# ipl-uw/ZeDO-Release

Measured on AMD Instinct MI355X. Metric: poses/sec (1000-step sampler, H=50), higher is better.
Workload: dtype f32; 1 GPU; BASELINE configs[2] (3DPW pw3d_test, H=50, 1000 steps): N=1015 poses/GPU x H=50 hypotheses, IPO 500 it (17 joints) + 1000 OIL steps + P1/P2 min-over-hypotheses selection; random-init ScoreModelFC_Adv weights, synthetic detections; settings=pw3d, rows_per_gpu=50750, poses_total=1015

## Files before the change

### zedo-release_amd/csrc/zedo_geom.hip

```cpp
#include "zedo_internal.h"

#include <atomic>
#include <cstdlib>

namespace zedo {


__global__ void pack_rows_kernel(const float *__restrict__ x, float *__restrict__ xpad, int B, int Bp, int D) {
    const size_t i = (size_t)blockIdx.x * blockDim.x + threadIdx.x;
    if (i >= (size_t)Bp * XLD) return;
    const int r = (int)(i / XLD), c = (int)(i % XLD);
#ifdef ZEDO_MUT_PACK51
    if (D > 51) D = 51;
#endif
    xpad[i] = (r < B && c < D) ? x[(size_t)r * D + c] : 0.0f;
}

__global__ void unpack_rows_kernel(const float *__restrict__ xpad, float *__restrict__ x, int B, int D) {
    const size_t i = (size_t)blockIdx.x * blockDim.x + threadIdx.x;
    if (i >= (size_t)B * D) return;
    const int r = (int)(i / D), c = (int)(i % D);
    x[i] = xpad[(size_t)r * XLD + c];
}

hipError_t launch_pack_rows(const float *x, float *xpad, int B, int Bp, int D, hipStream_t st) {
    const size_t n = (size_t)Bp * XLD;
    hipLaunchKernelGGL(pack_rows_kernel, dim3((unsigned)((n + 255) / 256)), dim3(256), 0, st, x, xpad, B, Bp, D);
    return hipGetLastError();
}
hipError_t launch_unpack_rows(const float *xpad, float *x, int B, int D, hipStream_t st) {
    const size_t n = (size_t)B * D;
    hipLaunchKernelGGL(unpack_rows_kernel, dim3((unsigned)((n + 255) / 256)), dim3(256), 0, st, xpad, x, B, D);
    return hipGetLastError();
}

__device__ __forceinline__ void inv3x3(const float *K, double *Ki) {
    const double a = K[0], b = K[1], c = K[2], d = K[3], e = K[4], f = K[5], g = K[6], h = K[7], i = K[8];
    const double A = e * i - f * h, Bc = -(d * i - f * g), C = d * h - e * g;
    const double det = a * A + b * Bc + c * C;
    const double id = 1.0 / det;
    Ki[0] = A * id;  Ki[1] = -(b * i - c * h) * id;  Ki[2] = (b * f - c * e) * id;
    Ki[3] = Bc * id; Ki[4] = (a * i - c * g) * id;   Ki[5] = -(a * f - c * d) * id;
    Ki[6] = C * id;  Ki[7] = -(a * h - b * g) * id;  Ki[8] = (a * e - b * d) * id;
}

__global__ void reproj_prepare_kernel(const float *__restrict__ uv, const float *__restrict__ K,
                                      const float *__restrict__ conf, int N, int J, float *__restrict__ geom,
                                      float *__restrict__ conf_out) {
    const int i = blockIdx.x * blockDim.x + threadIdx.x;
    if (i >= N * J) return;
    const int n = i / J;
    double Ki[9];
    inv3x3(K + (size_t)n * 9, Ki);
    const double u = uv[(size_t)i * 2], v = uv[(size_t)i * 2 + 1];
    const double rz = Ki[6] * u + Ki[7] * v + Ki[8];
    const double rx = (Ki[0] * u + Ki[1] * v + Ki[2]) / rz;
    const double ry = (Ki[3] * u + Ki[4] * v + Ki[5]) / rz;
    const double rn = 1.0 / sqrt(rx * rx + ry * ry + 1.0);
    float W = 1.0f;
    if (conf) {
        float c = conf[i];
        if (c > 1.0f) c = 1.0f;
        if (c < 1e-4f) c = 1e-4f;
        if (conf_out) conf_out[i] = c;
        const float w = c * c;
        W = w * w;
#ifdef ZEDO_MUT_CONF2
        W = w;
#endif
    }
    float *g = geom + (size_t)i * GEOM_F;
    g[0] = (float)rx; g[1] = (float)ry; g[2] = W; g[3] = 0.0f;
    g[4] = (float)(rx * rn); g[5] = (float)(ry * rn); g[6] = (float)rn; g[7] = 0.0f;
}

hipError_t launch_reproj_prepare(const float *uv, const float *K, const float *conf, int N, int J, float *geom,
                                 float *conf_clamped, hipStream_t st) {
    const int n = N * J;
    hipLaunchKernelGGL(reproj_prepare_kernel, dim3((n + 255) / 256), dim3(256), 0, st, uv, K, conf, N, J, geom,
                       conf_clamped);
    return hipGetLastError();
}

__global__ void reproj_degenerate_kernel(const float *__restrict__ geom, int N, int J, int *__restrict__ count) {
    const int n = blockIdx.x * blockDim.x + threadIdx.x;
    if (n >= N) return;
    const float *gp = geom + (size_t)n * J * GEOM_F;
    float sw = 0.f, srx = 0.f, sry = 0.f;
    for (int j = 0; j < J; ++j) {
        const f32x4 a = *reinterpret_cast<const f32x4 *>(gp + j * GEOM_F);
        sw += a[2]; srx += a[2] * a[0]; sry += a[2] * a[1];
    }
    const float iw = 1.0f / sw;
    const float mrx = srx * iw, mry = sry * iw;
    float den = 0.f;
    for (int j = 0; j < J; ++j) {
        const f32x4 a = *reinterpret_cast<const f32x4 *>(gp + j * GEOM_F);
        const float dx = a[0] - mrx, dy = a[1] - mry;
        den += a[2] * (dx * dx + dy * dy);
    }
    if (den == 0.f) atomicAdd(count, 1);
}

hipError_t launch_reproj_degenerate(const float *geom, int N, int J, int *d_count, hipStream_t st) {
    hipLaunchKernelGGL(reproj_degenerate_kernel, dim3((N + 255) / 256), dim3(256), 0, st, geom, N, J, d_count);
    return hipGetLastError();
}


template <int J>
__global__ __launch_bounds__(128) void reproj_grad_kernel(const float *__restrict__ x, const float *__restrict__ geom,
                                                          float *__restrict__ T, int solve, float *__restrict__ gout,
                                                          int B, int N, long long row_offset) {
    constexpr int D = J * 3, R = 128;
    __shared__ float sx[R * D];
    const int row0 = blockIdx.x * R, tid = threadIdx.x;
    const int rows = min(R, B - row0);
    const float *src = x + (size_t)row0 * D;
    for (int i = tid; i < rows * D; i += R) sx[i] = src[i];
    __syncthreads();
    float xr[D], gr[D], Tr[3];
    if (tid < rows) {
        const int b = row0 + tid;
#pragma unroll
        for (int c = 0; c < D; ++c) xr[c] = sx[tid * D + c];
        Tr[0] = T[(size_t)b * 3]; Tr[1] = T[(size_t)b * 3 + 1]; Tr[2] = T[(size_t)b * 3 + 2];
#ifdef ZEDO_MUT_RGRAD_OFFSET
        const int n = b % N;
#else
        const int n = (int)((row_offset + b) % N);
#endif
        reproj_row<J>(xr, geom + (size_t)n * J * GEOM_F, Tr, solve != 0, gr);
        if (solve) { T[(size_t)b * 3] = Tr[0]; T[(size_t)b * 3 + 1] = Tr[1]; T[(size_t)b * 3 + 2] = Tr[2]; }
    }
    __syncthreads();
    if (tid < rows) {
#pragma unroll
        for (int c = 0; c < D; ++c) sx[tid * D + c] = gr[c];
    }
    __syncthreads();
    float *dst = gout + (size_t)row0 * D;
    for (int i = tid; i < rows * D; i += R) dst[i] = sx[i];
}

hipError_t launch_reproj_grad(const float *x, const float *geom, float *T, int solve_T, float *g, int B, int N,
                              int J, long long row_offset, hipStream_t st) {
    if (J != 17) return hipErrorInvalidValue;
    hipLaunchKernelGGL(reproj_grad_kernel<17>, dim3((B + 127) / 128), dim3(128), 0, st, x, geom, T, solve_T, g, B, N,
                       row_offset);
    return hipGetLastError();
}

constexpr int TILE_LD = XLD + 4;
__device__ __forceinline__ void tile_to_lds(float *sx, const float *base, const int tid) {
#pragma unroll
    for (int it = 0; it < XLD / 4; ++it) {
        const int idx = it * BATCH_PAD + tid, r = idx >> 4, c4 = idx & 15;
        *reinterpret_cast<f32x4 *>(sx + r * TILE_LD + c4 * 4) = *reinterpret_cast<const f32x4 *>(base + (size_t)idx * 4);
    }
}
__device__ __forceinline__ void tile_from_lds(float *base, const float *sx, const int tid) {
#pragma unroll
    for (int it = 0; it < XLD / 4; ++it) {
        const int idx = it * BATCH_PAD + tid, r = idx >> 4, c4 = idx & 15;
        *reinterpret_cast<f32x4 *>(base + (size_t)idx * 4) = *reinterpret_cast<const f32x4 *>(sx + r * TILE_LD + c4 * 4);
    }
}

template <int J>
__global__ __launch_bounds__(64) void reproj_step_kernel(float *__restrict__ xpad, const float *__restrict__ geom,
                                                         float *__restrict__ T, int solve, int B, int N,
                                                         long long row_offset) {
    __shared__ __attribute__((aligned(16))) float sx[BATCH_PAD * TILE_LD];
    const int row0 = blockIdx.x * BATCH_PAD, tid = threadIdx.x;
    float *base = xpad + (size_t)row0 * XLD;
    tile_to_lds(sx, base, tid);
    __syncthreads();
    const int b = row0 + tid;
    if (b < B) ZEDO_REPROJ_STAGED_ROW(J, sx + tid * TILE_LD, 0, b, (ReprojArgs{geom, T, solve, B, N, row_offset}));
    __syncthreads();
    tile_from_lds(base, sx, tid);
}

template <int J>
__global__ __launch_bounds__(64) void post_reduce_kernel(float *__restrict__ xpad, const float *__restrict__ partial,
                                                         const float *__restrict__ bias, float sde_a, float sde_c, int sde,
                                                         float *__restrict__ eps_out, const float *__restrict__ geom,
                                                         float *__restrict__ T, int solve, int B, int N, long long row_offset) {
    __shared__ __attribute__((aligned(16))) float sx[BATCH_PAD * TILE_LD];
    __shared__ __attribute__((aligned(16))) float sb[XLD];
    const int row0 = blockIdx.x * BATCH_PAD, tid = threadIdx.x;
    float *base = (sde ? xpad : eps_out) + (size_t)row0 * XLD;
    sb[tid] = bias[tid];
    if (sde) tile_to_lds(sx, base, tid);
    __syncthreads();
    const int b = row0 + tid;
    {
        const float *p0 = partial + ((size_t)(b >> 5) * 4 * 32 + (b & 31)) * XLD;
        float *xr = sx + tid * TILE_LD;
#pragma unroll
        for (int v = 0; v < XLD / 4; ++v) {
            const f32x4 q0 = *reinterpret_cast<const f32x4 *>(p0 + v * 4);
            const f32x4 q1 = *reinterpret_cast<const f32x4 *>(p0 + 32 * XLD + v * 4);
            const f32x4 q2 = *reinterpret_cast<const f32x4 *>(p0 + 2 * 32 * XLD + v * 4);
#ifdef ZEDO_MUT_POST_Q3
            const f32x4 q3 = q2;
#else
            const f32x4 q3 = *reinterpret_cast<const f32x4 *>(p0 + 3 * 32 * XLD + v * 4);
#endif
            const f32x4 bb = *reinterpret_cast<const f32x4 *>(sb + v * 4);
            f32x4 x4 = {0.f, 0.f, 0.f, 0.f};
            if (sde) x4 = *reinterpret_cast<const f32x4 *>(xr + v * 4);
            f32x4 o;
#pragma unroll
            for (int e = 0; e < 4; ++e) {
                float t = ((q0[e] + q1[e]) + q2[e]) + q3[e];
                t = t + bb[e];
                if (sde) { t = t * sde_c; t = __builtin_fmaf(sde_a, x4[e], t); }
                o[e] = t;
            }
            *reinterpret_cast<f32x4 *>(xr + v * 4) = o;
        }
    }
    if (geom != nullptr && b < B) ZEDO_REPROJ_STAGED_ROW(J, sx + tid * TILE_LD, 0, b, (ReprojArgs{geom, T, solve, B, N, row_offset}));
    __syncthreads();
    tile_from_lds(base, sx, tid);
}

hipError_t launch_post_reduce(float *xpad, const float *partial, const float *bias, float sde_a, float sde_c, int sde,
                              float *eps_out, const ReprojArgs &rp, int Bp, hipStream_t st) {
    if (Bp % BATCH_PAD || !partial || !bias || (sde ? !xpad : !eps_out)) return hipErrorInvalidValue;
    hipLaunchKernelGGL(post_reduce_kernel<17>, dim3(Bp / BATCH_PAD), dim3(BATCH_PAD), 0, st, xpad, partial, bias, sde_a, sde_c, sde,
                       eps_out, rp.geom, rp.T, rp.solve, rp.B, rp.N > 0 ? rp.N : 1, rp.row0);
    return hipGetLastError();
}

hipError_t launch_reproj_step_padded(float *xpad, const ReprojArgs &rp, hipStream_t st) {
    hipLaunchKernelGGL(reproj_step_kernel<17>, dim3((rp.B + BATCH_PAD - 1) / BATCH_PAD), dim3(BATCH_PAD), 0, st, xpad, rp.geom, rp.T,
                       rp.solve, rp.B, rp.N, rp.row0);
    return hipGetLastError();
}

__global__ void posemb_kernel(const float *__restrict__ t, int S, int Sp, float label_scale, float *__restrict__ pe) {
    const int i = blockIdx.x * blockDim.x + threadIdx.x;
    if (i >= Sp * EMB) return;
    const int s = i / EMB, c = i % EMB;
    float o = 0.0f;
    if (s < S) {
        constexpr int half = EMB / 2;
        const float emb = (float)(-9.210340371976184 / (half - 1));
        const int k = c < half ? c : c - half;
        const float freq = expf((float)k * emb);
        const float arg = (t[s] * label_scale) * freq;
        o = c < half ? sinf(arg) : cosf(arg);
#ifdef ZEDO_MUT_POSEMB_FAST
        o = c < half ? __sinf(arg) : __cosf(arg);
#endif
    }
    pe[i] = o;
}

hipError_t launch_posemb(const float *t, int S, int Sp, float label_scale, float *pe, hipStream_t st) {
    const int n = Sp * EMB;
    hipLaunchKernelGGL(posemb_kernel, dim3((n + 255) / 256), dim3(256), 0, st, t, S, Sp, label_scale, pe);
    return hipGetLastError();
}

struct AdamP {
    float p, m, v;
    __device__ __forceinline__ void step(float g, float step_size, float bc2_sqrt) {
        m = m + (g - m) * 0.1f;
        v = v * 0.999f + 0.001f * g * g;
        const float denom = sqrtf(v) / bc2_sqrt + 1e-8f;
        p = p + (-step_size * m) / denom;
    }
};

__device__ __forceinline__ float sgnf(float e) { return (e > 0.f) ? 1.f : ((e < 0.f) ? -1.f : 0.f); }

constexpr int IPO_KMAX = 17;
static_assert(IPO_KMAX == 17, "launch_ipo_fit instantiates ipo_row_kernel<1 .. 17>: a longer key list needs its cases");
constexpr int IPO_TABLE = 2048;

struct IpoKeys { int j[IPO_KMAX]; };

__constant__ float c_adam_step[IPO_TABLE] = {
#define ZEDO_ADAM_STEP
#include "zedo_adam_table.inc"
#undef ZEDO_ADAM_STEP
};
__constant__ float c_adam_bc2s[IPO_TABLE] = {
#define ZEDO_ADAM_BC2S
#include "zedo_adam_table.inc"
#undef ZEDO_ADAM_BC2S
};

template <int M>
__device__ __forceinline__ float swz_xor(float v) {
    return __int_as_float(__builtin_amdgcn_ds_swizzle(__float_as_int(v), (M << 10) | 0x1F));
}
template <int CTRL>
__device__ __forceinline__ float dpp(float v) {
    return __int_as_float(__builtin_amdgcn_update_dpp(0, __float_as_int(v), CTRL, 0xF, 0xF, false));
}
template <int C>
__device__ __forceinline__ float bcast(float v) {
    return __int_as_float(__builtin_amdgcn_ds_swizzle(__float_as_int(v), (C << 5)));
}
__device__ __forceinline__ float half_sum(float v) {
    v = v + dpp<0x140>(v);
    v = v + dpp<0x141>(v);
    v = v + dpp<0x4E>(v);
    v = v + dpp<0xB1>(v);
    v = v + swz_xor<16>(v);
    return v;
}

struct IpoRot { float R00, R01, R02, R10, R11, R12, R20, R21, R22, Tx, Ty, Tz, ts; };

__device__ __forceinline__ IpoRot ipo_rot(float r, float i, float j, float kk, float scp, float min_s, float max_s, const float (&T0)[3]) {
    IpoRot o;
    const float n2 = r * r + i * i + j * j + kk * kk;
    const float ts = 2.0f / n2;
    o.ts = ts;
    o.R00 = 1.f - ts * (j * j + kk * kk); o.R01 = ts * (i * j - kk * r); o.R02 = ts * (i * kk + j * r);
    o.R10 = ts * (i * j + kk * r); o.R11 = 1.f - ts * (i * i + kk * kk); o.R12 = ts * (j * kk - i * r);
    o.R20 = ts * (i * kk - j * r); o.R21 = ts * (j * kk + i * r); o.R22 = 1.f - ts * (i * i + j * j);
    const float scc = fminf(fmaxf(scp, min_s), max_s);
    o.Tx = T0[0] * scc; o.Ty = T0[1] * scc; o.Tz = T0[2] * scc;
    return o;
}

__device__ __forceinline__ void ipo_joint_terms(const float (&K)[9], const float (&T0)[3], const IpoRot &o, float x, float y, float z,
                                                float cu, float cv, float inv_norm, float (&t)[10]) {
    const float px = o.R00 * x + o.R01 * y + o.R02 * z + o.Tx;
    const float py = o.R10 * x + o.R11 * y + o.R12 * z + o.Ty;
    const float pz = o.R20 * x + o.R21 * y + o.R22 * z + o.Tz;
    const float w0 = K[0] * px + K[1] * py + K[2] * pz;
    const float w1 = K[3] * px + K[4] * py + K[5] * pz;
#ifdef ZEDO_MUT_IPO_W2_K6
    const float w2 = K[7] * py + K[8] * pz;
#else
    const float w2 = K[6] * px + K[7] * py + K[8] * pz;
#endif
    const float gu = sgnf(w0 / w2 - cu) * inv_norm;
    const float gv = sgnf(w1 / w2 - cv) * inv_norm;
    const float gw0 = gu / w2, gw1 = gv / w2;
    const float gw2 = -gu * ((w0 / w2) / w2) - gv * ((w1 / w2) / w2);
    const float gpx = K[0] * gw0 + K[3] * gw1 + K[6] * gw2;
#ifdef ZEDO_MUT_IPO_GPY_K1
    const float gpy = K[4] * gw1 + K[7] * gw2;
#else
    const float gpy = K[1] * gw0 + K[4] * gw1 + K[7] * gw2;
#endif
    const float gpz = K[2] * gw0 + K[5] * gw1 + K[8] * gw2;
    t[0] = gpx * T0[0] + gpy * T0[1] + gpz * T0[2];
    t[1] = gpx * x; t[2] = gpx * y; t[3] = gpx * z;
    t[4] = gpy * x; t[5] = gpy * y; t[6] = gpy * z;
    t[7] = gpz * x; t[8] = gpz * y; t[9] = gpz * z;
}

__device__ __forceinline__ void ipo_quat_grads(const float (&S)[10], float r, float i, float j, float kk, float ts, float &gr, float &gi,
                                               float &gj, float &gk) {
    const float G00 = S[1], G01 = S[2], G02 = S[3], G10 = S[4], G11 = S[5], G12 = S[6], G20 = S[7], G21 = S[8], G22 = S[9];
    const float gts = G00 * -(j * j + kk * kk) + G01 * (i * j - kk * r) + G02 * (i * kk + j * r) +
                      G10 * (i * j + kk * r) + G11 * -(i * i + kk * kk) + G12 * (j * kk - i * r) +
                      G20 * (i * kk - j * r) + G21 * (j * kk + i * r) + G22 * -(i * i + j * j);
    const float dts = -gts * ts * ts;
    gr = ts * (-G01 * kk + G02 * j + G10 * kk - G12 * i - G20 * j + G21 * i) + dts * r;
    gi = ts * (G01 * j + G02 * kk + G10 * j - 2.f * G11 * i - G12 * r + G20 * kk + G21 * r - 2.f * G22 * i) + dts * i;
    gj = ts * (-2.f * G00 * j + G01 * i + G02 * r + G10 * i + G12 * kk - G20 * r + G21 * kk - 2.f * G22 * j) + dts * j;
    gk = ts * (-2.f * G00 * kk - G01 * r + G02 * i + G10 * r - 2.f * G11 * kk + G12 * j + G20 * i + G21 * j) + dts * kk;
}

__device__ __forceinline__ void ipo_T0(const float (&K)[9], double u, double v, float ipo_T, float (&T0)[3]) {
    double Ki[9];
    inv3x3(K, Ki);
    const double tx = Ki[0] * u + Ki[1] * v + Ki[2], ty = Ki[3] * u + Ki[4] * v + Ki[5], tz = Ki[6] * u + Ki[7] * v + Ki[8];
    const double in = (double)ipo_T / sqrt(tx * tx + ty * ty + tz * tz);
    T0[0] = (float)(tx * in); T0[1] = (float)(ty * in); T0[2] = (float)(tz * in);
}

__device__ __forceinline__ void ipo_adam_terms(int ta, double &b1p, double &b2p, float &step_size, float &bc2s) {
    b1p *= 0.9; b2p *= 0.999;
    if (ta < IPO_TABLE) { step_size = c_adam_step[ta]; bc2s = c_adam_bc2s[ta]; }
    else { step_size = (float)(0.1 / (1.0 - b1p)); bc2s = (float)sqrt(1.0 - b2p); }
}

__device__ __forceinline__ void ipo_store(const AdamP &qr, const AdamP &qi, const AdamP &qj, const AdamP &qk, const AdamP &sc, const float (&T0)[3],
                                          float min_s, float max_s, int b, float *Rout, float *Tout, float *qout, float *sout, float *stp) {
    const float r = qr.p, i = qi.p, j = qj.p, kk = qk.p;
    const float ts = 2.0f / (r * r + i * i + j * j + kk * kk);
    float *Ro = Rout + (size_t)b * 9;
    Ro[0] = 1.f - ts * (j * j + kk * kk); Ro[1] = ts * (i * j - kk * r); Ro[2] = ts * (i * kk + j * r);
    Ro[3] = ts * (i * j + kk * r); Ro[4] = 1.f - ts * (i * i + kk * kk); Ro[5] = ts * (j * kk - i * r);
    Ro[6] = ts * (i * kk - j * r); Ro[7] = ts * (j * kk + i * r); Ro[8] = 1.f - ts * (i * i + j * j);
    const float scc = fminf(fmaxf(sc.p, min_s), max_s);
    Tout[(size_t)b * 3] = T0[0] * scc; Tout[(size_t)b * 3 + 1] = T0[1] * scc; Tout[(size_t)b * 3 + 2] = T0[2] * scc;
    if (qout) { qout[(size_t)b * 4] = r; qout[(size_t)b * 4 + 1] = i; qout[(size_t)b * 4 + 2] = j; qout[(size_t)b * 4 + 3] = kk; }
    if (sout) sout[b] = sc.p;
    if (stp) {
        stp[0] = qr.p; stp[1] = qi.p; stp[2] = qj.p; stp[3] = qk.p; stp[4] = sc.p;
        stp[5] = qr.m; stp[6] = qi.m; stp[7] = qj.m; stp[8] = qk.m; stp[9] = sc.m;
#ifdef ZEDO_MUT_IPO_STORE_V
        stp[10] = qr.v; stp[11] = qi.v; stp[12] = qj.v; stp[13] = qk.v; stp[14] = sc.m;
#else
        stp[10] = qr.v; stp[11] = qi.v; stp[12] = qj.v; stp[13] = qk.v; stp[14] = sc.v;
#endif
    }
}

__global__ __launch_bounds__(64) void ipo_kernel(const float *__restrict__ x0, const float *__restrict__ uv,
                                                  const float *__restrict__ Kmat, const IpoKeys keylist,
                                                  int k, int axes_mask, float ipo_T, float min_s, float max_s,
                                                  int iters, float inv_norm, float *__restrict__ Rout,
                                                  float *__restrict__ Tout, float *__restrict__ qout,
                                                  float *__restrict__ sout, float *__restrict__ state,
                                                  int it_begin, double b1p0, double b2p0, int B, int N, int J,
                                                  long long row_offset) {
    __shared__ int s_kl[32];
    const int lane = threadIdx.x, jl = lane & 31;
    if (lane < 32) s_kl[lane] = lane < k ? keylist.j[lane] : keylist.j[0];
    __syncthreads();
    const int b_raw = blockIdx.x * 2 + (lane >> 5);
    const bool row_ok = b_raw < B;
    const int b = row_ok ? b_raw : B - 1;
#ifdef ZEDO_MUT_IPO_JOINT
    const bool jact = jl < k && jl < 16;
#else
    const bool jact = jl < k;
#endif
    const long long gb = row_offset + b;
    const int n = (int)(gb % N), h = (int)(gb / N);
    const int jn = s_kl[jl];
    const float *xh = x0 + ((size_t)h * J + jn) * 3;
    const float x = xh[0], y = xh[1], z = xh[2];
    const float cu = uv[((size_t)n * J + jn) * 2], cv = uv[((size_t)n * J + jn) * 2 + 1];
    float K[9];
#pragma unroll
    for (int i = 0; i < 9; ++i) K[i] = Kmat[(size_t)n * 9 + i];
    float T0[3];
    ipo_T0(K, uv[(size_t)n * J * 2], uv[(size_t)n * J * 2 + 1], ipo_T, T0);
    AdamP qr{1.f, 0.f, 0.f}, qi{0.f, 0.f, 0.f}, qj{0.f, 0.f, 0.f}, qk{0.f, 0.f, 0.f}, sc{1.f, 0.f, 0.f};
#ifdef ZEDO_MUT_IPO_AXIS_XY
    const bool ax = axes_mask & 1, ay = axes_mask & 1, az = axes_mask & 4;
#else
    const bool ax = axes_mask & 1, ay = axes_mask & 2, az = axes_mask & 4;
#endif
    float *stp = state ? state + (size_t)b * 15 : nullptr;
    if (stp && it_begin > 0) {
        qr = AdamP{stp[0], stp[5], stp[10]}; qi = AdamP{stp[1], stp[6], stp[11]}; qj = AdamP{stp[2], stp[7], stp[12]};
        qk = AdamP{stp[3], stp[8], stp[13]}; sc = AdamP{stp[4], stp[9], stp[14]};
    }
    double b1p = b1p0, b2p = b2p0;
    AdamP mine;
    mine.p = jl == 0 ? qr.p : jl == 1 ? qi.p : jl == 2 ? qj.p : jl == 3 ? qk.p : sc.p;
    mine.m = jl == 0 ? qr.m : jl == 1 ? qi.m : jl == 2 ? qj.m : jl == 3 ? qk.m : sc.m;
    mine.v = jl == 0 ? qr.v : jl == 1 ? qi.v : jl == 2 ? qj.v : jl == 3 ? qk.v : sc.v;
    for (int it = 0; it < iters; ++it) {
        const float r = qr.p, i = qi.p, j = qj.p, kk = qk.p;
        const IpoRot o = ipo_rot(r, i, j, kk, sc.p, min_s, max_s, T0);
        float t[10], S[10];
        ipo_joint_terms(K, T0, o, x, y, z, cu, cv, inv_norm, t);
#pragma unroll
        for (int e = 0; e < 10; ++e) S[e] = half_sum(jact ? t[e] : 0.f);
        float gr, gi, gj, gk;
        ipo_quat_grads(S, r, i, j, kk, o.ts, gr, gi, gj, gk);
#ifdef ZEDO_MUT_IPO_CLAMP_LO
        const float gs = (sc.p <= max_s) ? S[0] : 0.f;
#else
        const float gs = (sc.p >= min_s && sc.p <= max_s) ? S[0] : 0.f;
#endif
        float step_size, bc2s;
        ipo_adam_terms(it_begin + it, b1p, b2p, step_size, bc2s);
        {
            const float g_c = jl == 0 ? gr : jl == 1 ? gi : jl == 2 ? gj : jl == 3 ? gk : gs;
            const bool upd = jl == 0 || (jl == 1 && ax) || (jl == 2 && ay) || (jl == 3 && az) || jl == 4;
            AdamP nxt = mine;
            nxt.step(g_c, step_size, bc2s);
            if (upd) mine = nxt;
            qr.p = bcast<0>(mine.p); qi.p = bcast<1>(mine.p); qj.p = bcast<2>(mine.p); qk.p = bcast<3>(mine.p); sc.p = bcast<4>(mine.p);
        }
    }
    qr.m = bcast<0>(mine.m); qi.m = bcast<1>(mine.m); qj.m = bcast<2>(mine.m); qk.m = bcast<3>(mine.m); sc.m = bcast<4>(mine.m);
    qr.v = bcast<0>(mine.v); qi.v = bcast<1>(mine.v); qj.v = bcast<2>(mine.v); qk.v = bcast<3>(mine.v); sc.v = bcast<4>(mine.v);
    if (row_ok && jl == 0) ipo_store(qr, qi, qj, qk, sc, T0, min_s, max_s, b, Rout, Tout, qout, sout, stp);
}

constexpr int IPO_ROW_TB = 128;
template <int KJ, int S>
__device__ __forceinline__ void ipo_slot(const float (&K)[9], const float (&T0)[3], const IpoRot &o, const float (&x)[KJ], const float (&y)[KJ],
                                         const float (&z)[KJ], const float *cu, const float *cv, float inv_norm, float (&t)[10]) {
#ifdef ZEDO_MUT_IPO_JOINT
    constexpr bool live = S < KJ && S < 16;
#else
    constexpr bool live = S < KJ;
#endif
    if constexpr (live) {
        ipo_joint_terms(K, T0, o, x[S], y[S], z[S], cu[S * IPO_ROW_TB], cv[S * IPO_ROW_TB], inv_norm, t);
    } else {
#pragma unroll
        for (int e = 0; e < 10; ++e) t[e] = 0.f;
    }
}
#define IPO_SLOT_ARGS K, T0, o, x, y, z, cu, cv, inv_norm
#define IPO_SLOT_PARAMS const float (&K)[9], const float (&T0)[3], const IpoRot &o, const float (&x)[KJ], const float (&y)[KJ], \
                        const float (&z)[KJ], const float *cu, const float *cv, float inv_norm
template <int KJ, int BASE, int I>
__device__ __forceinline__ void ipo_pair_a(IPO_SLOT_PARAMS, float (&a)[10]) {
    float u[10], v[10];
    ipo_slot<KJ, BASE + I>(IPO_SLOT_ARGS, u);
    ipo_slot<KJ, BASE + 15 - I>(IPO_SLOT_ARGS, v);
#pragma unroll
    for (int e = 0; e < 10; ++e) a[e] = u[e] + v[e];
}
template <int KJ, int BASE, int I>
__device__ __forceinline__ void ipo_pair_b(IPO_SLOT_PARAMS, float (&b)[10]) {
    float u[10], v[10];
    ipo_pair_a<KJ, BASE, I>(IPO_SLOT_ARGS, u);
    ipo_pair_a<KJ, BASE, 7 - I>(IPO_SLOT_ARGS, v);
#pragma unroll
    for (int e = 0; e < 10; ++e) b[e] = u[e] + v[e];
}
template <int KJ, int BASE>
__device__ __forceinline__ void ipo_row_sum(IPO_SLOT_PARAMS, float (&d)[10]) {
    float b0[10], b1[10], b2[10], b3[10];
    ipo_pair_b<KJ, BASE, 0>(IPO_SLOT_ARGS, b0);
    ipo_pair_b<KJ, BASE, 2>(IPO_SLOT_ARGS, b2);
#pragma unroll
    for (int e = 0; e < 10; ++e) b0[e] = b0[e] + b2[e];
    ipo_pair_b<KJ, BASE, 1>(IPO_SLOT_ARGS, b1);
    ipo_pair_b<KJ, BASE, 3>(IPO_SLOT_ARGS, b3);
#pragma unroll
    for (int e = 0; e < 10; ++e) d[e] = b0[e] + (b1[e] + b3[e]);
}

template <int KJ>
__global__ __launch_bounds__(IPO_ROW_TB) void ipo_row_kernel(const float *__restrict__ x0, const float *__restrict__ uv,
                                                             const float *__restrict__ Kmat, const IpoKeys keylist, int axes_mask,
                                                             float ipo_T, float min_s, float max_s, int iters, float inv_norm,
                                                             float *__restrict__ Rout, float *__restrict__ Tout,
                                                             float *__restrict__ qout, float *__restrict__ sout,
                                                             float *__restrict__ state, int it_begin, double b1p0, double b2p0,
                                                             int B, int N, int J, long long row_offset) {
    __shared__ float s_cu[KJ][IPO_ROW_TB], s_cv[KJ][IPO_ROW_TB];
    const int tid = threadIdx.x;
    const int b = blockIdx.x * IPO_ROW_TB + tid;
    if (b >= B) return;
    const long long gb = row_offset + b;
    const int n = (int)(gb % N), h = (int)(gb / N);
    float x[KJ], y[KJ], z[KJ];
#pragma unroll
    for (int jj = 0; jj < KJ; ++jj) {
        const int jn = keylist.j[jj];
        const float *xh = x0 + ((size_t)h * J + jn) * 3;
        x[jj] = xh[0]; y[jj] = xh[1]; z[jj] = xh[2];
        s_cu[jj][tid] = uv[((size_t)n * J + jn) * 2];
        s_cv[jj][tid] = uv[((size_t)n * J + jn) * 2 + 1];
    }
    const float *cu = &s_cu[0][tid], *cv = &s_cv[0][tid];
    float K[9];
#pragma unroll
    for (int i = 0; i < 9; ++i) K[i] = Kmat[(size_t)n * 9 + i];
    float T0[3];
    ipo_T0(K, uv[(size_t)n * J * 2], uv[(size_t)n * J * 2 + 1], ipo_T, T0);
    AdamP qr{1.f, 0.f, 0.f}, qi{0.f, 0.f, 0.f}, qj{0.f, 0.f, 0.f}, qk{0.f, 0.f, 0.f}, sc{1.f, 0.f, 0.f};
#ifdef ZEDO_MUT_IPO_AXIS_XY
    const bool ax = axes_mask & 1, ay = axes_mask & 1, az = axes_mask & 4;
#else
    const bool ax = axes_mask & 1, ay = axes_mask & 2, az = axes_mask & 4;
#endif
    float *stp = state ? state + (size_t)b * 15 : nullptr;
    if (stp && it_begin > 0) {
        qr = AdamP{stp[0], stp[5], stp[10]}; qi = AdamP{stp[1], stp[6], stp[11]}; qj = AdamP{stp[2], stp[7], stp[12]};
        qk = AdamP{stp[3], stp[8], stp[13]}; sc = AdamP{stp[4], stp[9], stp[14]};
#ifdef ZEDO_MUT_IPO_ROW_LOAD_V
        qr.v = qi.v = qj.v = qk.v = sc.v = 0.f;
#endif
    }
    double b1p = b1p0, b2p = b2p0;
    for (int it = 0; it < iters; ++it) {
        const float r = qr.p, i = qi.p, j = qj.p, kk = qk.p;
        const IpoRot o = ipo_rot(r, i, j, kk, sc.p, min_s, max_s, T0);
        float d0[10], d1[10], S[10];
        ipo_row_sum<KJ, 0>(IPO_SLOT_ARGS, d0);
        ipo_row_sum<KJ, 16>(IPO_SLOT_ARGS, d1);
#pragma unroll
        for (int e = 0; e < 10; ++e) S[e] = d0[e] + d1[e];
        float gr, gi, gj, gk;
        ipo_quat_grads(S, r, i, j, kk, o.ts, gr, gi, gj, gk);
#ifdef ZEDO_MUT_IPO_CLAMP_LO
        const float gs = (sc.p <= max_s) ? S[0] : 0.f;
#else
        const float gs = (sc.p >= min_s && sc.p <= max_s) ? S[0] : 0.f;
#endif
        float step_size, bc2s;
        ipo_adam_terms(it_begin + it, b1p, b2p, step_size, bc2s);
        qr.step(gr, step_size, bc2s);
        if (ax) qi.step(gi, step_size, bc2s);
        if (ay) qj.step(gj, step_size, bc2s);
        if (az) qk.step(gk, step_size, bc2s);
        sc.step(gs, step_size, bc2s);
    }
    ipo_store(qr, qi, qj, qk, sc, T0, min_s, max_s, b, Rout, Tout, qout, sout, stp);
}
#undef IPO_SLOT_ARGS
#undef IPO_SLOT_PARAMS

hipError_t launch_ipo_fit(const float *x0, const float *uv, const float *K, const int *h_keylist, int k,
                          int axes_mask, float ipo_T, float min_scale, float max_scale, int iters,
                          double normaliser, float *R, float *T, float *q, float *scale, float *state, int it_begin,
                          int B, int N, int J, long long row_offset, hipStream_t st) {
    if (k < 1 || k > IPO_KMAX) return hipErrorInvalidValue;
    double b1p0 = 1.0, b2p0 = 1.0;
    for (int i = 0; i < it_begin; ++i) { b1p0 *= 0.9; b2p0 *= 0.999; }
    IpoKeys keys{};
    for (int i = 0; i < k; ++i) keys.j[i] = h_keylist[i];
    static const char *pin = getenv("ZEDO_IPO_KERNEL");
    bool row = B >= num_cus() * (k == 17 ? 68 : 4 * k + 4);
    if (pin && pin[0] == 'h') row = false;
    if (pin && pin[0] == 'r') row = true;
    const float inv_norm = (float)(1.0 / normaliser);
    if (row) {
        const dim3 grid((B + IPO_ROW_TB - 1) / IPO_ROW_TB), block(IPO_ROW_TB);
#define ZEDO_IPO_ROW_CASE(KJ)                                                                                                                   \
        case KJ:                                                                                                                                \
            hipLaunchKernelGGL(ipo_row_kernel<KJ>, grid, block, 0, st, x0, uv, K, keys, axes_mask, ipo_T, min_scale, max_scale, iters, inv_norm, R, T, \
                               q, scale, state, it_begin, b1p0, b2p0, B, N, J, row_offset);                                                    \
            break;
        switch (k) {
            ZEDO_IPO_ROW_CASE(1) ZEDO_IPO_ROW_CASE(2) ZEDO_IPO_ROW_CASE(3) ZEDO_IPO_ROW_CASE(4) ZEDO_IPO_ROW_CASE(5) ZEDO_IPO_ROW_CASE(6)
            ZEDO_IPO_ROW_CASE(7) ZEDO_IPO_ROW_CASE(8) ZEDO_IPO_ROW_CASE(9) ZEDO_IPO_ROW_CASE(10) ZEDO_IPO_ROW_CASE(11) ZEDO_IPO_ROW_CASE(12)
            ZEDO_IPO_ROW_CASE(13) ZEDO_IPO_ROW_CASE(14) ZEDO_IPO_ROW_CASE(15) ZEDO_IPO_ROW_CASE(16) ZEDO_IPO_ROW_CASE(17)
            default: return hipErrorInvalidValue;
        }
#undef ZEDO_IPO_ROW_CASE
        return hipGetLastError();
    }
    hipLaunchKernelGGL(ipo_kernel, dim3((B + 1) / 2), dim3(64), 0, st, x0, uv, K, keys, k,
                       axes_mask, ipo_T, min_scale, max_scale, iters, inv_norm, R, T, q, scale, state,
                       it_begin, b1p0, b2p0, B, N, J, row_offset);
    return hipGetLastError();
}

__global__ void rotate_init_kernel(const float *__restrict__ x0, const float *__restrict__ R, float *__restrict__ x,
                                   int B, int N, int J, long long row_offset) {
    const size_t i = (size_t)blockIdx.x * blockDim.x + threadIdx.x;
    if (i >= (size_t)B * J) return;
    const int b = (int)(i / J), j = (int)(i % J);
    const int h = (int)((row_offset + b) / N);
    const float *r = R + (size_t)b * 9;
    const float *p = x0 + ((size_t)h * J + j) * 3;
    const float a = p[0], c = p[1], d = p[2];
    x[i * 3] = r[0] * a + r[1] * c + r[2] * d;
    x[i * 3 + 1] = r[3] * a + r[4] * c + r[5] * d;
    x[i * 3 + 2] = r[6] * a + r[7] * c + r[8] * d;
}

hipError_t launch_rotate_init(const float *x0, const float *R, float *x, int B, int N, int J, long long row_offset,
                              hipStream_t st) {
    const size_t n = (size_t)B * J;
    hipLaunchKernelGGL(rotate_init_kernel, dim3((unsigned)((n + 255) / 256)), dim3(256), 0, st, x0, R, x, B, N, J,
                       row_offset);
    return hipGetLastError();
}

}
```

Measured before the change: 320.8 poses/s.

## Split IPO row fit across 2/4 lanes per row with DPP reductions and LDS z

Reworks the row-per-thread IPO kernel so each row can be split across 1, 2 or 4 lanes. Each lane handles a subset of the joints and the partial gradient sums are combined with DPP cross-lane adds. A 'slim' variant moves the z coordinates into LDS and raises launch bounds to allow 2 blocks per CU, and the block size grows to 256. Launch heuristics choose the lane count from B relative to CU count. The aim is better occupancy and parallelism for the 500-iteration IPO fit, at the cost of more complex templates and duplicated per-lane Adam work.

New measurement: 320.9 poses/s (median of 2 runs). About the same (+0.0%).

```diff
diff --git a/zedo-release_amd/csrc/zedo_geom.hip b/zedo-release_amd/csrc/zedo_geom.hip
--- a/zedo-release_amd/csrc/zedo_geom.hip
+++ b/zedo-release_amd/csrc/zedo_geom.hip
@@ -2,6 +2,7 @@
 
 #include <atomic>
 #include <cstdlib>
+#include <cstring>
 
 namespace zedo {
 
@@ -487,78 +488,136 @@
     if (row_ok && jl == 0) ipo_store(qr, qi, qj, qk, sc, T0, min_s, max_s, b, Rout, Tout, qout, sout, stp);
 }
 
-constexpr int IPO_ROW_TB = 128;
-template <int KJ, int S>
-__device__ __forceinline__ void ipo_slot(const float (&K)[9], const float (&T0)[3], const IpoRot &o, const float (&x)[KJ], const float (&y)[KJ],
-                                         const float (&z)[KJ], const float *cu, const float *cv, float inv_norm, float (&t)[10]) {
+constexpr int IPO_ROW_TB = 256;
+template <int NX, bool LDS> struct IpoZ;
+template <int NX> struct IpoZ<NX, false> {
+    float v[NX];
+    template <int AT> __device__ __forceinline__ float get() const { return v[AT]; }
+    template <int AT> __device__ __forceinline__ void set(float a) { v[AT] = a; }
+};
+template <int NX> struct IpoZ<NX, true> {
+    float *p;
+    template <int AT> __device__ __forceinline__ float get() const { return p[AT * IPO_ROW_TB]; }
+    template <int AT> __device__ __forceinline__ void set(float a) { p[AT * IPO_ROW_TB] = a; }
+};
+constexpr bool ipo_owned(int S, int L) {
+    return S >= 16 || L == 1 || (L == 2 ? ((S ^ (S >> 2)) & 1) == 0 : ((S & 7) == 0 || (S & 7) == 7));
+}
+constexpr int ipo_first(int S, int L) { return S < 16 ? (S & ~(L - 1)) : S; }
+constexpr int ipo_last(int S, int L) { return S < 16 ? (S | (L - 1)) : S; }
+constexpr bool ipo_has(int KJ, int S, int L) { return ipo_owned(S, L) && ipo_first(S, L) < KJ; }
+constexpr int ipo_at(int KJ, int S, int L) {
+    int c = 0;
+    for (int s = 0; s < S; ++s) c += ipo_has(KJ, s, L);
+    return c;
+}
+constexpr int ipo_nx(int KJ, int L) { return ipo_at(KJ, 32, L); }
+#define IPO_SLOT_ARGS K, T0, o, x, y, z, cu, cv, inv_norm, q
+#define IPO_SLOT_PARAMS const float (&K)[9], const float (&T0)[3], const IpoRot &o, const float (&x)[ipo_nx(KJ, L)],                 \
+                        const float (&y)[ipo_nx(KJ, L)], const Z &z, const float *cu, const float *cv,                               \
+                        float inv_norm, int q
+template <int KJ, int L, int S, class Z>
+__device__ __forceinline__ void ipo_slot(IPO_SLOT_PARAMS, float (&t)[10]) {
 #ifdef ZEDO_MUT_IPO_JOINT
-    constexpr bool live = S < KJ && S < 16;
-#else
-    constexpr bool live = S < KJ;
+    constexpr bool live = ipo_has(KJ, S, L) && S < 16;
+#else
+    constexpr bool live = ipo_has(KJ, S, L);
 #endif
     if constexpr (live) {
-        ipo_joint_terms(K, T0, o, x[S], y[S], z[S], cu[S * IPO_ROW_TB], cv[S * IPO_ROW_TB], inv_norm, t);
+        constexpr int at = ipo_at(KJ, S, L);
+        ipo_joint_terms(K, T0, o, x[at], y[at], z.template get<at>(), cu[at * IPO_ROW_TB], cv[at * IPO_ROW_TB], inv_norm, t);
+        if constexpr (ipo_last(S, L) >= KJ) {
+            const bool mine = (S ^ q) < KJ;
+#pragma unroll
+            for (int e = 0; e < 10; ++e) t[e] = mine ? t[e] : 0.f;
+        }
     } else {
 #pragma unroll
         for (int e = 0; e < 10; ++e) t[e] = 0.f;
     }
 }
-#define IPO_SLOT_ARGS K, T0, o, x, y, z, cu, cv, inv_norm
-#define IPO_SLOT_PARAMS const float (&K)[9], const float (&T0)[3], const IpoRot &o, const float (&x)[KJ], const float (&y)[KJ], \
-                        const float (&z)[KJ], const float *cu, const float *cv, float inv_norm
-template <int KJ, int BASE, int I>
+template <int KJ, int L, int BASE, int I, class Z>
 __device__ __forceinline__ void ipo_pair_a(IPO_SLOT_PARAMS, float (&a)[10]) {
     float u[10], v[10];
-    ipo_slot<KJ, BASE + I>(IPO_SLOT_ARGS, u);
-    ipo_slot<KJ, BASE + 15 - I>(IPO_SLOT_ARGS, v);
+    ipo_slot<KJ, L, BASE + I>(IPO_SLOT_ARGS, u);
+    ipo_slot<KJ, L, BASE + 15 - I>(IPO_SLOT_ARGS, v);
 #pragma unroll
     for (int e = 0; e < 10; ++e) a[e] = u[e] + v[e];
 }
-template <int KJ, int BASE, int I>
+template <int KJ, int L, int BASE, int I, class Z>
 __device__ __forceinline__ void ipo_pair_b(IPO_SLOT_PARAMS, float (&b)[10]) {
     float u[10], v[10];
-    ipo_pair_a<KJ, BASE, I>(IPO_SLOT_ARGS, u);
-    ipo_pair_a<KJ, BASE, 7 - I>(IPO_SLOT_ARGS, v);
+    ipo_pair_a<KJ, L, BASE, I>(IPO_SLOT_ARGS, u);
+    ipo_pair_a<KJ, L, BASE, 7 - I>(IPO_SLOT_ARGS, v);
 #pragma unroll
     for (int e = 0; e < 10; ++e) b[e] = u[e] + v[e];
 }
-template <int KJ, int BASE>
+template <int KJ, int L, int BASE, class Z>
 __device__ __forceinline__ void ipo_row_sum(IPO_SLOT_PARAMS, float (&d)[10]) {
-    float b0[10], b1[10], b2[10], b3[10];
-    ipo_pair_b<KJ, BASE, 0>(IPO_SLOT_ARGS, b0);
-    ipo_pair_b<KJ, BASE, 2>(IPO_SLOT_ARGS, b2);
-#pragma unroll
-    for (int e = 0; e < 10; ++e) b0[e] = b0[e] + b2[e];
-    ipo_pair_b<KJ, BASE, 1>(IPO_SLOT_ARGS, b1);
-    ipo_pair_b<KJ, BASE, 3>(IPO_SLOT_ARGS, b3);
-#pragma unroll
-    for (int e = 0; e < 10; ++e) d[e] = b0[e] + (b1[e] + b3[e]);
-}
-
-template <int KJ>
-__global__ __launch_bounds__(IPO_ROW_TB) void ipo_row_kernel(const float *__restrict__ x0, const float *__restrict__ uv,
+    float b0[10];
+    ipo_pair_b<KJ, L, BASE, 0>(IPO_SLOT_ARGS, b0);
+    if constexpr (L == 4 && BASE == 0) {
+#pragma unroll
+        for (int e = 0; e < 10; ++e) b0[e] = b0[e] + dpp<0x4E>(b0[e]);
+    } else {
+        float b2[10];
+        ipo_pair_b<KJ, L, BASE, 2>(IPO_SLOT_ARGS, b2);
+#pragma unroll
+        for (int e = 0; e < 10; ++e) b0[e] = b0[e] + b2[e];
+    }
+    if constexpr (L > 1 && BASE == 0) {
+#pragma unroll
+        for (int e = 0; e < 10; ++e) d[e] = b0[e] + dpp<0xB1>(b0[e]);
+    } else {
+        float b1[10], b3[10];
+        ipo_pair_b<KJ, L, BASE, 1>(IPO_SLOT_ARGS, b1);
+        ipo_pair_b<KJ, L, BASE, 3>(IPO_SLOT_ARGS, b3);
+#pragma unroll
+        for (int e = 0; e < 10; ++e) d[e] = b0[e] + (b1[e] + b3[e]);
+    }
+}
+
+template <int KJ, int L, int S = 0, class Z>
+__device__ __forceinline__ void ipo_load(const float *xh, const float *uvn, const IpoKeys &keylist, int q, float (&x)[ipo_nx(KJ, L)],
+                                         float (&y)[ipo_nx(KJ, L)], Z &z, float *cu, float *cv) {
+    if constexpr (S <= IPO_KMAX) {
+        if constexpr (ipo_has(KJ, S, L)) {
+            constexpr int at = ipo_at(KJ, S, L);
+            int jn = keylist.j[S < KJ ? S : 0];
+            if constexpr (S < 16) {
+#pragma unroll
+                for (int qq = 1; qq < L; ++qq)
+                    if (q == qq) jn = keylist.j[(S ^ qq) < KJ ? (S ^ qq) : 0];
+            }
+            x[at] = xh[jn * 3]; y[at] = xh[jn * 3 + 1]; z.template set<at>(xh[jn * 3 + 2]);
+            cu[at * IPO_ROW_TB] = uvn[jn * 2];
+            cv[at * IPO_ROW_TB] = uvn[jn * 2 + 1];
+        }
+        ipo_load<KJ, L, S + 1>(xh, uvn, keylist, q, x, y, z, cu, cv);
+    }
+}
+
+template <int KJ, int L, bool ZLDS>
+__global__ __launch_bounds__(IPO_ROW_TB, ZLDS ? 2 : 1) void ipo_row_kernel(const float *__restrict__ x0, const float *__restrict__ uv,
                                                              const float *__restrict__ Kmat, const IpoKeys keylist, int axes_mask,
                                                              float ipo_T, float min_s, float max_s, int iters, float inv_norm,
                                                              float *__restrict__ Rout, float *__restrict__ Tout,
                                                              float *__restrict__ qout, float *__restrict__ sout,
                                                              float *__restrict__ state, int it_begin, double b1p0, double b2p0,
                                                              int B, int N, int J, long long row_offset) {
-    __shared__ float s_cu[KJ][IPO_ROW_TB], s_cv[KJ][IPO_ROW_TB];
-    const int tid = threadIdx.x;
-    const int b = blockIdx.x * IPO_ROW_TB + tid;
-    if (b >= B) return;
+    constexpr int NX = ipo_nx(KJ, L);
+    __shared__ float s_cu[NX][IPO_ROW_TB], s_cv[NX][IPO_ROW_TB], s_cz[ZLDS ? NX : 1][IPO_ROW_TB];
+    const int tid = threadIdx.x, q = tid & (L - 1);
+    const long long b_raw = ((long long)blockIdx.x * IPO_ROW_TB + tid) / L;
+    if (b_raw >= B) return;
+    const int b = (int)b_raw;
     const long long gb = row_offset + b;
     const int n = (int)(gb % N), h = (int)(gb / N);
-    float x[KJ], y[KJ], z[KJ];
-#pragma unroll
-    for (int jj = 0; jj < KJ; ++jj) {
-        const int jn = keylist.j[jj];
-        const float *xh = x0 + ((size_t)h * J + jn) * 3;
-        x[jj] = xh[0]; y[jj] = xh[1]; z[jj] = xh[2];
-        s_cu[jj][tid] = uv[((size_t)n * J + jn) * 2];
-        s_cv[jj][tid] = uv[((size_t)n * J + jn) * 2 + 1];
-    }
-    const float *cu = &s_cu[0][tid], *cv = &s_cv[0][tid];
+    float x[NX], y[NX];
+    IpoZ<NX, ZLDS> z;
+    if constexpr (ZLDS) z.p = &s_cz[0][tid];
+    float *cu = &s_cu[0][tid], *cv = &s_cv[0][tid];
+    ipo_load<KJ, L>(x0 + (size_t)h * J * 3, uv + (size_t)n * J * 2, keylist, q, x, y, z, cu, cv);
     float K[9];
 #pragma unroll
     for (int i = 0; i < 9; ++i) K[i] = Kmat[(size_t)n * 9 + i];
@@ -582,9 +641,10 @@
     for (int it = 0; it < iters; ++it) {
         const float r = qr.p, i = qi.p, j = qj.p, kk = qk.p;
         const IpoRot o = ipo_rot(r, i, j, kk, sc.p, min_s, max_s, T0);
+        if constexpr (ZLDS) asm volatile("" ::: "memory");
         float d0[10], d1[10], S[10];
-        ipo_row_sum<KJ, 0>(IPO_SLOT_ARGS, d0);
-        ipo_row_sum<KJ, 16>(IPO_SLOT_ARGS, d1);
+        ipo_row_sum<KJ, L, 0>(IPO_SLOT_ARGS, d0);
+        ipo_row_sum<KJ, L, 16>(IPO_SLOT_ARGS, d1);
 #pragma unroll
         for (int e = 0; e < 10; ++e) S[e] = d0[e] + d1[e];
         float gr, gi, gj, gk;
@@ -602,10 +662,12 @@
         if (az) qk.step(gk, step_size, bc2s);
         sc.step(gs, step_size, bc2s);
     }
-    ipo_store(qr, qi, qj, qk, sc, T0, min_s, max_s, b, Rout, Tout, qout, sout, stp);
+    if (q == 0) ipo_store(qr, qi, qj, qk, sc, T0, min_s, max_s, b, Rout, Tout, qout, sout, stp);
 }
 #undef IPO_SLOT_ARGS
 #undef IPO_SLOT_PARAMS
+
+constexpr int IPO_SLIM_FROM = 14;
 
 hipError_t launch_ipo_fit(const float *x0, const float *uv, const float *K, const int *h_keylist, int k,
                           int axes_mask, float ipo_T, float min_scale, float max_scale, int iters,
@@ -617,16 +679,29 @@
     IpoKeys keys{};
     for (int i = 0; i < k; ++i) keys.j[i] = h_keylist[i];
     static const char *pin = getenv("ZEDO_IPO_KERNEL");
-    bool row = B >= num_cus() * (k == 17 ? 68 : 4 * k + 4);
-    if (pin && pin[0] == 'h') row = false;
-    if (pin && pin[0] == 'r') row = true;
+    const int cus = num_cus();
+    int lanes = B < cus * (k + 5) ? 0 : B <= cus * (IPO_ROW_TB / 4) ? 4 : B <= cus * (IPO_ROW_TB / 2) ? 2 : 1;
+    bool slim = k == IPO_KMAX || (k >= IPO_SLIM_FROM && B > cus * IPO_ROW_TB);
+    if (pin && *pin) {
+        slim = k >= IPO_SLIM_FROM && !strcmp(pin, "slim");
+        if (!strcmp(pin, "half")) lanes = 0;
+        else if (!strcmp(pin, "row") || !strcmp(pin, "slim")) lanes = 1;
+        else if (!strcmp(pin, "pair")) lanes = 2;
+        else if (!strcmp(pin, "quad")) lanes = 4;
+        else return hipErrorInvalidValue;
+    }
     const float inv_norm = (float)(1.0 / normaliser);
-    if (row) {
-        const dim3 grid((B + IPO_ROW_TB - 1) / IPO_ROW_TB), block(IPO_ROW_TB);
+    if (lanes) {
+        const dim3 grid((unsigned)(((long long)B * lanes + IPO_ROW_TB - 1) / IPO_ROW_TB)), block(IPO_ROW_TB);
+#define ZEDO_IPO_ROW_LAUNCH(KJ, L, ZLDS)                                                                                                        \
+            hipLaunchKernelGGL((ipo_row_kernel<KJ, L, ZLDS>), grid, block, 0, st, x0, uv, K, keys, axes_mask, ipo_T, min_scale, max_scale, iters,    \
+                               inv_norm, R, T, q, scale, state, it_begin, b1p0, b2p0, B, N, J, row_offset)
 #define ZEDO_IPO_ROW_CASE(KJ)                                                                                                                   \
         case KJ:                                                                                                                                \
-            hipLaunchKernelGGL(ipo_row_kernel<KJ>, grid, block, 0, st, x0, uv, K, keys, axes_mask, ipo_T, min_scale, max_scale, iters, inv_norm, R, T, \
-                               q, scale, state, it_begin, b1p0, b2p0, B, N, J, row_offset);                                                    \
+            if (lanes == 4) ZEDO_IPO_ROW_LAUNCH(KJ, 4, false);                                                                                  \
+            else if (lanes == 2) ZEDO_IPO_ROW_LAUNCH(KJ, 2, false);                                                                             \
+            else if (slim) ZEDO_IPO_ROW_LAUNCH(KJ, 1, (KJ >= IPO_SLIM_FROM));                                                                   \
+            else ZEDO_IPO_ROW_LAUNCH(KJ, 1, false);                                                                                             \
             break;
         switch (k) {
             ZEDO_IPO_ROW_CASE(1) ZEDO_IPO_ROW_CASE(2) ZEDO_IPO_ROW_CASE(3) ZEDO_IPO_ROW_CASE(4) ZEDO_IPO_ROW_CASE(5) ZEDO_IPO_ROW_CASE(6)
@@ -635,6 +710,7 @@
             default: return hipErrorInvalidValue;
         }
 #undef ZEDO_IPO_ROW_CASE
+#undef ZEDO_IPO_ROW_LAUNCH
         return hipGetLastError();
     }
     hipLaunchKernelGGL(ipo_kernel, dim3((B + 1) / 2), dim3(64), 0, st, x0, uv, K, keys, k,
```
